# pinellolab/GRAFIMO

Hardware: AMD Instinct MI355X
Metric: scored haplotype k-mers/sec (higher is better)
Workload: dtype int32

## Files before the change

### grafimo_amd/_native.py

```python
import ctypes
import os

import numpy as np

_HERE = os.path.dirname(os.path.abspath(__file__))
LIB_PATH = os.environ.get("GRAFIMO_HIP_LIB") or os.path.join(_HERE, "csrc", "libgrafimo_hip.so")

GFM_OK = 0
GFM_ERR_INVALID = -1
GFM_ERR_ASSERT = -2
GFM_ERR_HIP = -3
GFM_ERR_NOMEM = -4
GFM_ERR_NODEVICE = -5
GFM_ERR_IO = -6
GFM_ERR_OVERFLOW = -7
GFM_NO_SELECT = 2**31 - 1
GFM_FLAG_RESET_HITS = 1
GFM_FLAG_CLEAR_HIST = 2
GFM_FLAG_CALLER_ORDERS_REUSE = 4
GFM_MAX_WIDTH = 64
GFM_BEST_ROW_BITS = 44
GFM_GRAPH_FORWARD_ONLY = 1
GFM_TSV_NO_NODEPATH = 1
GFM_WORKSPACE_RING = 4
GFM_HITS_DROP_ZERO_FREQ = 1
GFM_HITS_FIRST_PER_REGION = 2
GFM_VARIANT_ALL_SITES = 1
GFM_VARIANT_KEEP_ZERO_FREQ = 2
GFM_PAIRS_HAVE_OFFSETS = 1
GFM_LINKAGE_HAVE_OFFSETS = 1
GFM_SEQS_HAVE_LENGTHS = 1
ABI_VERSION = 12
RANGE = 1000

c_int = ctypes.c_int
c_i32 = ctypes.c_int32
c_i64 = ctypes.c_int64
c_u64 = ctypes.c_uint64
c_double = ctypes.c_double
c_void_p = ctypes.c_void_p
P = ctypes.POINTER

PROTOTYPES = {
    "gfm_abi_version": (c_int, []),
    "gfm_last_error": (ctypes.c_char_p, []),
    "gfm_device_count": (c_int, [P(c_int)]),
    "gfm_set_device": (c_int, [c_int]),
    "gfm_compute_log_odds": (c_int, [c_void_p, c_int, c_void_p, c_void_p]),
    "gfm_scale_pwm": (c_int, [c_void_p, c_int, c_void_p, P(c_int), P(c_int), P(c_int), P(c_double)]),
    "gfm_comp_pval_mat": (c_int, [c_void_p, c_int, c_void_p, c_void_p]),
    "gfm_comp_pval_mat_many": (c_int, [c_int, c_void_p, c_void_p, c_void_p, c_void_p]),
    "gfm_motif_create": (c_int, [c_void_p, c_int, c_void_p, c_int, c_int, c_double, c_void_p, P(c_void_p)]),
    "gfm_motif_create_many": (c_int, [c_int, c_void_p, c_void_p, c_void_p, c_void_p, c_void_p, c_void_p, c_void_p,
                                      c_void_p]),
    "gfm_motif_destroy": (None, [c_void_p]),
    "gfm_motif_width": (c_int, [c_void_p]),
    "gfm_motif_table_len": (c_int, [c_void_p]),
    "gfm_motif_score_range": (c_int, [c_void_p, P(c_i32), P(c_i32)]),
    "gfm_motif_tables": (c_int, [c_void_p, c_void_p, c_void_p]),
    "gfm_motif_pvalue_cutoff": (c_int, [c_void_p, c_double, P(c_i32)]),
    "gfm_motif_annotate": (c_int, [c_void_p, c_void_p, c_i64, c_void_p, c_void_p]),
    "gfm_score_kmers": (c_int, [c_void_p, c_void_p, c_i64, c_void_p, c_void_p, c_i32, c_i64,
                                c_void_p, c_i64, c_void_p, ctypes.c_uint32, c_void_p, c_void_p]),
    "gfm_score_kmers_multi": (c_int, [c_void_p, c_int, c_void_p, c_i64, c_void_p, c_void_p, c_void_p, c_i64,
                                      c_void_p, c_void_p, c_void_p, ctypes.c_uint32, c_void_p]),
    "gfm_score_kmers_multi_plan": (c_int, [c_void_p, c_int, c_void_p, c_void_p, c_void_p]),
    "gfm_profile_enable": (c_int, [c_void_p, c_int, c_int]),
    "gfm_profile_read": (c_int, [c_void_p, c_void_p, c_int, P(c_int)]),
    "gfm_profile_mark_tail": (c_int, [c_void_p, c_void_p]),
    "gfm_profile_read_tail": (c_int, [c_void_p, c_void_p, c_int, P(c_int)]),
    "gfm_calibrate_stream": (c_int, [c_int, c_i64, c_int, c_int, P(c_double), P(c_double)]),
    "gfm_qvalue_table": (c_int, [c_void_p, c_void_p, c_double, c_int, c_void_p, c_void_p, c_void_p,
                                 ctypes.c_uint32, c_void_p]),
    "gfm_qvalue_table_multi": (c_int, [c_void_p, c_int, c_void_p, c_double, c_int, c_void_p, c_void_p, c_void_p,
                                       ctypes.c_uint32, c_void_p]),
    "gfm_select_hits": (c_int, [c_void_p, c_void_p, c_i64, c_void_p, c_i64, c_void_p, c_i64, c_void_p,
                                ctypes.c_uint32, c_void_p]),
    "gfm_select_hits_from": (c_int, [c_void_p, c_void_p, c_i64, c_void_p, c_i64, c_void_p, c_i64, c_void_p,
                                     c_void_p, c_i64, c_void_p, c_void_p]),
    "gfm_region_ids": (c_int, [c_void_p, c_i32, c_i64, c_void_p, c_void_p]),
    "gfm_region_best": (c_int, [c_void_p, c_i64, c_void_p, c_i32, c_void_p, c_i32, c_void_p, c_i64, c_void_p, c_void_p]),
    "gfm_locus_max_workspace": (c_i64, [c_i64]),
    "gfm_locus_max": (c_int, [c_void_p, c_i64, c_void_p, c_i32, c_void_p, c_void_p, c_void_p, c_i32, c_void_p, c_void_p,
                              c_i64, c_void_p, c_void_p]),
    "gfm_scan_host": (c_int, [c_void_p, c_void_p, c_i64, c_double, c_int, c_int, c_i64, c_void_p,
                              c_void_p, c_void_p, c_void_p, c_void_p, P(c_i64)]),
    "gfm_tsv_open": (c_int, [P(ctypes.c_char_p), c_int, c_int, c_int, c_int, P(c_void_p), P(c_i64)]),
    "gfm_tsv_count_rows": (c_int, [ctypes.c_char_p, c_int, P(c_i64)]),
    "gfm_tsv_read": (c_int, [c_void_p] * 9),
    "gfm_tsv_name_count": (c_int, [c_void_p]),
    "gfm_tsv_names_bytes": (c_i64, [c_void_p]),
    "gfm_tsv_names": (c_int, [c_void_p, c_void_p, c_void_p]),
    "gfm_tsv_close": (None, [c_void_p]),
    "gfm_scan_tsv": (c_int, [c_void_p, P(ctypes.c_char_p), c_int, c_int, c_int, c_double, c_int, c_int, c_i64,
                             P(c_void_p), P(c_i64), P(c_i64)]),
    "gfm_scan_tsv_begin": (c_int, [c_void_p, c_int, P(ctypes.c_char_p), c_int, c_int, c_int, c_double, c_int, c_int,
                                   c_i64, c_void_p, P(c_void_p), P(c_i64)]),
    "gfm_scan_tsv_finish": (c_int, [c_void_p, c_void_p]),
# ... 174 lines not shown
```

### grafimo_amd/csrc/grafimo_hip.hip

```cpp

#include <hip/hip_runtime.h>

#include <algorithm>
#include <atomic>
#include <cmath>
#include <cstdarg>
#include <cstdint>
#include <cstdio>
#include <cstdlib>
#include <cstring>
#include <new>
#include <string>
#include <vector>

#include "grafimo_hip.h"

#define GFM_API extern "C" __attribute__((visibility("default")))

#include "gfm_hit_sort.hpp"
#include "gfm_common.hpp"
#include "gfm_score_kernels.hpp"
#include "gfm_quad_launch.hpp"
#include "gfm_stats_kernels.hpp"

// ... 7 lines not shown
    struct Window { int bins, lo; double mass; };
    std::vector<Window> windows;
    int device = 0;
    int n_cu = 256;
    int max_slabs = 0;
    int sel_slabs = 0;
    int reserve_cus = kReserveCUs;
    size_t lds_bytes = 0;
    std::vector<int64_t> sm;
    double bg[4] = {0, 0, 0, 0};
    std::vector<double> h_ptable;
    unsigned char *d_slab = nullptr;
    uint16_t *d_tab = nullptr;
    unsigned *d_ftab = nullptr;
    double *d_pmf = nullptr;
    double *d_ptable = nullptr;
    unsigned *d_partials[kWorkspaces] = {};
    unsigned *d_spill[kWorkspaces] = {};
    long long *d_resid[kWorkspaces] = {};
    int *d_resid_n[kWorkspaces] = {};
    QWork *d_qwork = nullptr;
    double *d_qscratch = nullptr;
    hipStream_t q_stream[kQStreams] = {};
    int q_streams_used = 0;
    unsigned long long q_last_use[kQStreams] = {}, q_calls = 0;
    hipEvent_t ev_selected = nullptr;
    hipStream_t sel_last_stream = nullptr;
    bool sel_valid = false;
    HitCtl *d_ctl = nullptr;
    unsigned call_no = 0;
    hipStream_t last_st = nullptr, last_tail = nullptr;
    unsigned same_pair_run = 0;
    hipEvent_t ev_scored[kWorkspaces] = {};
    hipEvent_t ev_posted[kWorkspaces] = {};
    bool posted_valid[kWorkspaces] = {};
    long long *d_sel_resid = nullptr;
    int *d_sel_resid_n = nullptr;
    HitCtl *d_sel_ctl = nullptr;
    unsigned sel_call_no = 0;
    std::vector<hipEvent_t> ev0, ev1;
    int ev_next = 0, ev_used = 0, ev_every = 1;
    unsigned ev_calls = 0;
    std::vector<hipEvent_t> tev0, tev1;
    int ev_last = -1;
    int tail_pending = -1;
    std::vector<int> tail_order;
};

namespace {

int ensure_device()
{
    int n = 0;
    hipError_t e = hipGetDeviceCount(&n);
    if (e != hipSuccess || n <= 0) {
        (void)hipGetLastError();
        return fail(GFM_ERR_NODEVICE, "no HIP device available (%s)",
                    e == hipSuccess ? "device count is 0" : hipGetErrorString(e));
    }
    return GFM_OK;
}

void cumulative_windows(const int64_t *sm, int W, std::vector<int> &lo, std::vector<int> &hi)
{
    lo.resize(W);
    hi.resize(W);
// ... 149 lines not shown
    q.hit_rows = d_hit_rows; q.hit_count = d_hit_count; q.hit_cap = cap;
    q.nslabs = hist_slabs; q.nb = win_nb; q.lo = win_lo; q.min_val = m->min_val;
    q.spill_lo = m->lo; q.spill_n = m->nb; q.hit_slabs = hit_slabs; q.par = ctl_slot;
    return q;
}

int launch_posts(const PostJob *jobs, int count, hipStream_t st)
{
    PostJobs all{};
    int live = 0, max_total = 0;
    for (int k = 0; k < count; ++k) {
        const PostJob &q = jobs[k];
        if (q.total == 0) {
            if (q.ctl)
                HIP_TRY(hipMemsetAsync(&q.ctl->mid[(q.par + kCtlAhead) % kCtlSlots], 0, sizeof(unsigned long long), st));
            continue;
        }
        all.j[live++] = q;
        max_total = std::max(max_total, q.total);
    }
    if (live == 0) return GFM_OK;
    hipLaunchKernelGGL(post_kernel, dim3((unsigned)max_total, (unsigned)live), dim3(256), 0, st, all);
    HIP_TRY(hipGetLastError());
    return GFM_OK;
}

int launch_post(gfm_motif *m, const unsigned *partials, int hist_slabs, unsigned long long *d_hist,
                int win_lo, int win_nb, unsigned *spill, const long long *resid, const int *resid_n, int hit_slabs, HitCtl *ctl, int ctl_slot,
                long long *d_hit_rows, long long cap, unsigned long long *d_hit_count, hipStream_t st)
{
    const PostJob q = post_job(m, partials, hist_slabs, d_hist, win_lo, win_nb, spill, resid, resid_n, hit_slabs, ctl,
                               ctl_slot, d_hit_rows, cap, d_hit_count);
    return launch_posts(&q, 1, st);
}

void fill_motif_args(MotifArgs &a, gfm_motif *m, int ws, int slot, int use_hist, int win_lo, int win_nb,
                     int cutoff,
                     int *d_scores, long long *d_hit_rows, long long cap,
                     const unsigned long long *d_hit_count_or_null)
{
    a.tab = m->d_tab;
    a.lo = win_lo;
    a.nb = win_nb;
    a.min_val = m->min_val;
    a.use_hist = use_hist;
    a.spill_lo = m->lo;
    a.spill_n = m->nb;
    a.spill = m->d_spill[ws];
    a.cutoff = cutoff;
    a.slot = slot;
    a.scores = d_scores;
    a.partials = m->d_partials[ws];
    a.hit_rows = d_hit_rows;
    a.hit_cap = cap;
    a.hit_count = d_hit_count_or_null;
    a.ctl = m->d_ctl;
    a.resid = m->d_resid[ws];
    a.resid_n = m->d_resid_n[ws];
}

bool plan_group(const gfm_motif_t *motifs, int n_left, const bool *with_hist, int *mm_out, int *waves_out,
                int *win_lo, int *win_nb)
{
    constexpr double kMinWindowMass = 0.999;
    const int W = motifs[0]->W;
    int mm = std::min(W <= kQuadMaxBatchWidth ? 3 : 1, n_left);
// ... 353 lines not shown
    double *rows = reinterpret_cast<double *>(d.p + rows_at), *pmfs = reinterpret_cast<double *>(d.p + pmf_at);
    size_t off = 0;
    for (DpJob &j : pk.jobs) {
        j.buf = rows + 2 * off;
        j.pmf = pmfs + off;
        off += (size_t)j.L;
    }
    img = pk.image();
    HIP_TRY(hipMemcpyAsync(d.p, img.data(), img.size(), hipMemcpyHostToDevice, nullptr));
    rc = pk.launch(d.p, n_motifs, false, nullptr);
    if (rc) return rc;
    HIP_TRY(hipMemcpy(h_pmf_out, pmfs, sizeof(double) * total_L, hipMemcpyDeviceToHost));
    return GFM_OK;
}

GFM_API int gfm_comp_pval_mat(const int64_t *sm, int W, const double *bg, double *h_pmf)
{
    return gfm_comp_pval_mat_many(1, sm, &W, bg, h_pmf);
}

GFM_API void gfm_motif_destroy(gfm_motif_t m)
{
    if (!m) return;
    if (m->d_slab) (void)hipFree(m->d_slab);
    for (int i = 0; i < kWorkspaces; ++i) {
        if (m->ev_scored[i]) (void)hipEventDestroy(m->ev_scored[i]);
        if (m->ev_posted[i]) (void)hipEventDestroy(m->ev_posted[i]);
    }
    for (auto e : m->ev0) (void)hipEventDestroy(e);
    for (auto e : m->ev1) (void)hipEventDestroy(e);
    for (auto e : m->tev0) (void)hipEventDestroy(e);
    for (auto e : m->tev1) (void)hipEventDestroy(e);
    if (m->ev_selected) (void)hipEventDestroy(m->ev_selected);
    delete m;
}

GFM_API int gfm_motif_create_many(int n_motifs, const int64_t *h_score_matrices, const int *widths, const double *h_bgs,
                                  const int *min_vals, const int *scales, const double *offsets,
                                  const double *const *h_pmfs, gfm_motif_t *out)
{
    if (n_motifs < 0) return fail(GFM_ERR_INVALID, "negative motif count %d", n_motifs);
    if (!out) return fail(GFM_ERR_INVALID, "NULL argument");
    for (int i = 0; i < n_motifs; ++i) out[i] = nullptr;
    if (n_motifs == 0) return GFM_OK;
    if (!h_score_matrices || !widths || !h_bgs || !min_vals || !scales || !offsets)
        return fail(GFM_ERR_INVALID, "NULL argument");
    std::vector<size_t> sm_at((size_t)n_motifs);
    size_t at = 0;
    for (int i = 0; i < n_motifs; ++i) {
        sm_at[(size_t)i] = at;
        const int rc = validate_motif(i, h_score_matrices + at, widths[i], h_bgs + 4 * (size_t)i, &min_vals[i], &scales[i]);
        if (rc) return rc;
        at += 4 * (size_t)widths[i];
    }
    int rc = ensure_device();
    if (rc) return rc;

    std::vector<std::vector<uint16_t>> tabs((size_t)n_motifs);
    std::vector<std::vector<unsigned>> ftabs((size_t)n_motifs);
    std::vector<unsigned char> img;
    DevBuf<unsigned char> d_pack;
    std::vector<gfm_motif *> ms((size_t)n_motifs, nullptr);
    auto bail = [&](int code) {
        (void)hipStreamSynchronize(nullptr);
        for (gfm_motif *m : ms) gfm_motif_destroy(m);
        return code;
// ... 82 lines not shown
        const int mid = (a + b) / 2;
        if (m->h_ptable[mid] < threshold) b = mid; else a = mid + 1;
    }
    *cutoff = a;
    return GFM_OK;
}

GFM_API int gfm_motif_annotate(gfm_motif_t m, const int32_t *scores, int64_t n, double *lo_out,
                               double *p_out)
{
    if (!m || (!scores && n)) return fail(GFM_ERR_INVALID, "NULL argument");
    for (int64_t i = 0; i < n; ++i) {
        const int s = scores[i];
        if (s < 0 || s >= m->L) return fail(GFM_ERR_INVALID, "score %d outside the table", s);
        if (lo_out) lo_out[i] = ((double)s / (double)m->scale) + ((double)m->W * m->offset);
        if (p_out) p_out[i] = m->h_ptable[s];
    }
    return GFM_OK;
}

GFM_API int gfm_score_kmers(gfm_motif_t m, const uint8_t *d_kmers, int64_t n, int32_t *d_scores,
                            uint64_t *d_hist, int32_t select_cutoff, int64_t row_base,
                            int64_t *d_hit_rows, int64_t hit_capacity, uint64_t *d_hit_count,
                            uint32_t flags, void *stream, void *tail_stream)
{
    if (!m) return fail(GFM_ERR_INVALID, "motif is NULL");
    if (n < 0) return fail(GFM_ERR_INVALID, "negative row count");
    hipStream_t st = static_cast<hipStream_t>(stream);
    hipStream_t tail = tail_stream ? static_cast<hipStream_t>(tail_stream) : st;
    const bool split = tail != st;
    if (n == 0) {
        if ((flags & GFM_FLAG_RESET_HITS) && d_hit_count) {
            if (split) {
                HIP_TRY(hipEventRecord(m->ev_scored[0], st));
                HIP_TRY(hipStreamWaitEvent(tail, m->ev_scored[0], 0));
            }
            HIP_TRY(hipMemsetAsync(d_hit_count, 0, sizeof(uint64_t), tail));
        }
        return GFM_OK;
    }
    if (!d_kmers) return fail(GFM_ERR_INVALID, "NULL device buffer");
    {
        int dev = -1;
        HIP_TRY(hipGetDevice(&dev));
        if (dev != m->device)
            return fail(GFM_ERR_INVALID, "the motif lives on device %d, the current device is %d", m->device, dev);
    }
    if ((reinterpret_cast<uintptr_t>(d_kmers) & 15u) != 0)
        return fail(GFM_ERR_INVALID, "d_kmers must be 16-byte aligned");
    if ((reinterpret_cast<uintptr_t>(d_scores) & 3u) != 0)
        return fail(GFM_ERR_INVALID, "d_scores must be 4-byte aligned");
    if (!d_scores && !d_hist && select_cutoff == GFM_NO_SELECT)
        return fail(GFM_ERR_INVALID, "nothing to do: no scores, no histogram, no selection");
    if (n > (int64_t)kQuadRows * 0x7fffff00ll)
        return fail(GFM_ERR_INVALID, "too many rows for one launch (split the batch)");
    const bool select = select_cutoff != GFM_NO_SELECT;
    if (select && (!d_hit_rows || !d_hit_count))
        return fail(GFM_ERR_INVALID, "selection requested without hit buffers");
    const int use_hist = d_hist ? 1 : 0;
    const long long nchunks = (n + kQuadRows - 1) / kQuadRows;
    const long long want = (nchunks + m->q_waves - 1) / m->q_waves;
    const int avail = split ? std::max(1, m->max_slabs - m->reserve_cus * (m->max_slabs / m->n_cu)) : m->max_slabs;
    int nslabs = (int)std::min<long long>(want, avail);
    if (want > avail) {
        long long best_cap = -1;
        for (int g = avail; g >= std::max(1, avail - avail / 8); --g) {
            const long long per_turn = (long long)g * m->q_waves;
            const long long cap = (nchunks + per_turn - 1) / per_turn * per_turn;
            if (best_cap < 0 || cap < best_cap) { best_cap = cap; nslabs = g; }
        }
#ifdef GFM_LAB
        if (const char *e = std::getenv("GRAFIMO_SCORE_GRID")) {
            const int g = atoi(e);
            if (g >= 1 && g <= m->max_slabs) nslabs = g;
        }
#endif
    }

    const unsigned k = m->call_no++;
    const int ws = (int)(k % (unsigned)kWorkspaces), slot = (int)(k % (unsigned)kCtlSlots);
    const int ws_prev = (int)((k + kWorkspaces - 1) % (unsigned)kWorkspaces);
    const bool reset = (flags & GFM_FLAG_RESET_HITS) != 0;
    const bool same_owner = st == m->last_st && tail == m->last_tail;
    const bool caller_orders = (flags & GFM_FLAG_CALLER_ORDERS_REUSE) && same_owner && m->same_pair_run >= (unsigned)kWorkspaces;
    m->same_pair_run = same_owner ? m->same_pair_run + 1 : 1;
    m->last_st = st;
    m->last_tail = tail;
    if (m->posted_valid[ws] && !caller_orders)
        HIP_TRY(hipStreamWaitEvent(st, m->ev_posted[ws], 0));
    if (split && select && !reset && m->posted_valid[ws_prev])
        HIP_TRY(hipStreamWaitEvent(st, m->ev_posted[ws_prev], 0));
    ScoreArgs<1> args{};
    args.store_through = d_scores ? score_store_through(n, 1) : 2;
    fill_motif_args(args.m[0], m, ws, slot, use_hist, m->hlo, m->hnb, select_cutoff, d_scores,
                    reinterpret_cast<long long *>(d_hit_rows), hit_capacity,
                    reset ? nullptr : reinterpret_cast<unsigned long long *>(d_hit_count));
    hipEvent_t scored = split ? m->ev_scored[ws] : nullptr;
    int rc = dispatch_quad(m->W, 1, m, d_kmers, n, row_base, &args, m->lds_bytes, nslabs, m->q_waves, st, false,
                           split ? &scored : nullptr);
    if (rc) return rc;
    if (split) HIP_TRY(hipStreamWaitEvent(tail, scored, 0));
    m->tail_pending = -1;
    if (split && m->ev_last >= 0 && !m->tev0.empty()) {
        HIP_TRY(hipEventRecord(m->tev0[m->ev_last], tail));
        m->tail_pending = m->ev_last;
    }
    rc = launch_post(m, m->d_partials[ws], nslabs, reinterpret_cast<unsigned long long *>(d_hist),
                     m->hlo, m->hnb, m->d_spill[ws], m->d_resid[ws], m->d_resid_n[ws], select ? nslabs : 0, m->d_ctl, slot,
                     reinterpret_cast<long long *>(d_hit_rows), hit_capacity,
                     reinterpret_cast<unsigned long long *>(d_hit_count), tail);
    if (rc) return rc;
    if (split) {
        HIP_TRY(hipEventRecord(m->ev_posted[ws], tail));
        m->posted_valid[ws] = true;
    } else {
        m->posted_valid[ws] = false;
    }
    return GFM_OK;
}

GFM_API int gfm_score_kmers_multi(const gfm_motif_t *motifs, int n_motifs, const uint8_t *d_kmers,
                                  int64_t n, int32_t *const *d_scores, uint64_t *const *d_hist,
                                  const int32_t *select_cutoffs, int64_t row_base,
                                  int64_t *const *d_hit_rows, const int64_t *hit_capacity,
                                  uint64_t *const *d_hit_count, uint32_t flags, void *stream)
{
    if (!motifs || n_motifs < 1) return fail(GFM_ERR_INVALID, "NULL argument");
    if (n < 0) return fail(GFM_ERR_INVALID, "negative row count");
    hipStream_t st = static_cast<hipStream_t>(stream);
    const bool reset = (flags & GFM_FLAG_RESET_HITS) != 0;
    bool no_scores = d_scores == nullptr;
    if (d_scores) {
        int n_null = 0;
// ... 27 lines not shown
        if ((reinterpret_cast<uintptr_t>(d_scores[i]) & 3u) != 0)
            return fail(GFM_ERR_INVALID, "d_scores[%d] must be 4-byte aligned", i);
    const int W = motifs[0]->W;
    const long long nchunks = (n + kQuadRows - 1) / kQuadRows;

    int i = 0;
    while (i < n_motifs) {
        int mm = 0, waves = kWavesPerWG, nb_lds[3] = {0, 0, 0};
        int win_lo[3] = {0, 0, 0}, win_nb[3] = {0, 0, 0};
        bool with_hist[3];
        for (int k = 0; k < 3; ++k) with_hist[k] = i + k < n_motifs && d_hist && d_hist[i + k];
        if (!plan_group(motifs + i, n_motifs - i, with_hist, &mm, &waves, win_lo, win_nb))
            return fail(GFM_ERR_INVALID, "no LDS left for a histogram window at width %d", W);
        for (int k = 0; k < mm; ++k) {
            if (win_nb[k] > motifs[i + k]->part_nb)
                return fail(GFM_ERR_INVALID, "internal error: histogram window larger than the workspace");
            nb_lds[k] = (d_hist && d_hist[i + k]) ? win_nb[k] + 1 : 0;
        }
        size_t lds = quad_fixed_lds(W, waves, mm);
        for (int k = 0; k < mm; ++k) lds += sizeof(unsigned) * (size_t)nb_lds[k];
        const long long want = (nchunks + waves - 1) / waves;
        int nslabs = (int)std::min<long long>(want, motifs[i]->max_slabs);
        for (int k = 1; k < mm; ++k) nslabs = std::min(nslabs, motifs[i + k]->max_slabs);
        int ws[3], slot[3], uh[3];
        ScoreArgs<1> a1{};
        ScoreArgs<2> a2{};
        ScoreArgs<3> a3{};
        a1.store_through = a2.store_through = a3.store_through = no_scores ? 2 : score_store_through(n, mm);
        for (int k = 0; k < mm; ++k) {
            gfm_motif *mo = motifs[i + k];
            const unsigned c = mo->call_no++;
            mo->same_pair_run = 0;
            mo->last_st = mo->last_tail = nullptr;
            ws[k] = (int)(c % (unsigned)kWorkspaces);
            slot[k] = (int)(c % (unsigned)kCtlSlots);
            mo->posted_valid[ws[k]] = false;
            uh[k] = (d_hist && d_hist[i + k]) ? 1 : 0;
            const int cut = select_cutoffs ? select_cutoffs[i + k] : GFM_NO_SELECT;
            const bool sel = cut != GFM_NO_SELECT;
            MotifArgs &dst = mm == 1 ? a1.m[k] : (mm == 2 ? a2.m[k] : a3.m[k]);
            fill_motif_args(dst, mo, ws[k], slot[k], uh[k], win_lo[k], win_nb[k], cut, no_scores ? nullptr : d_scores[i + k],
                            sel ? reinterpret_cast<long long *>(d_hit_rows[i + k]) : nullptr,
                            sel ? hit_capacity[i + k] : 0,
                            (sel && !reset) ? reinterpret_cast<const unsigned long long *>(d_hit_count[i + k])
                                            : nullptr);
        }
        const void *args = mm == 1 ? static_cast<const void *>(&a1) : (mm == 2 ? static_cast<const void *>(&a2) : &a3);
        int rc = dispatch_quad(W, mm, motifs[i], d_kmers, n, row_base, args, lds, nslabs, waves, st, false);
        if (rc) return rc;
        PostJob posts[kPostJobs];
        for (int k = 0; k < mm; ++k) {
            gfm_motif *mo = motifs[i + k];
            const int cut = select_cutoffs ? select_cutoffs[i + k] : GFM_NO_SELECT;
            const bool sel = cut != GFM_NO_SELECT;
            posts[k] = post_job(mo, mo->d_partials[ws[k]], nslabs,
                                uh[k] ? reinterpret_cast<unsigned long long *>(d_hist[i + k]) : nullptr,
                                win_lo[k], win_nb[k], mo->d_spill[ws[k]], mo->d_resid[ws[k]], mo->d_resid_n[ws[k]],
                                sel ? nslabs : 0, mo->d_ctl, slot[k],
                                sel ? reinterpret_cast<long long *>(d_hit_rows[i + k]) : nullptr,
                                sel ? hit_capacity[i + k] : 0,
                                sel ? reinterpret_cast<unsigned long long *>(d_hit_count[i + k]) : nullptr);
        }
        rc = launch_posts(posts, mm, st);
        if (rc) return rc;
        i += mm;
    }
    return GFM_OK;
}

GFM_API int gfm_score_kmers_multi_plan(const gfm_motif_t *motifs, int n_motifs, const int32_t *with_hist,
                                       int32_t *group_size_out, int32_t *waves_out)
{
    if (!motifs || n_motifs < 1) return fail(GFM_ERR_INVALID, "NULL argument");
    for (int i = 0; i < n_motifs; ++i) {
        if (!motifs[i]) return fail(GFM_ERR_INVALID, "motif %d is NULL", i);
        if (motifs[i]->W != motifs[0]->W)
            return fail(GFM_ERR_INVALID, "motifs of one batched launch must share their width (%d vs %d)",
                        motifs[i]->W, motifs[0]->W);
    }
    int i = 0;
    while (i < n_motifs) {
        int mm = 0, waves = 0, win_lo[3], win_nb[3];
        bool wh[3];
        for (int k = 0; k < 3; ++k) wh[k] = i + k < n_motifs && (!with_hist || with_hist[i + k]);
        if (!plan_group(motifs + i, n_motifs - i, wh, &mm, &waves, win_lo, win_nb))
            return fail(GFM_ERR_INVALID, "no LDS left for a histogram window at width %d", motifs[0]->W);
        for (int k = 0; k < mm; ++k) {
            if (group_size_out) group_size_out[i + k] = mm;
            if (waves_out) waves_out[i + k] = waves;
        }
        i += mm;
    }
    return GFM_OK;
}

GFM_API int gfm_profile_enable(gfm_motif_t m, int slots, int every)
{
    if (!m || slots < 0 || every < 1) return fail(GFM_ERR_INVALID, "bad argument");
    m->ev_every = every;
    m->ev_calls = 0;
    for (auto e : m->ev0) (void)hipEventDestroy(e);
    for (auto e : m->ev1) (void)hipEventDestroy(e);
    for (auto e : m->tev0) (void)hipEventDestroy(e);
    for (auto e : m->tev1) (void)hipEventDestroy(e);
    m->ev0.clear();
    m->ev1.clear();
    m->tev0.clear();
    m->tev1.clear();
    m->tail_order.clear();
    m->ev_next = m->ev_used = 0;
    m->ev_last = m->tail_pending = -1;
    for (int i = 0; i < slots; ++i) {
        hipEvent_t a, b, c, d;
        HIP_TRY(hipEventCreate(&a));
        HIP_TRY(hipEventCreate(&b));
        HIP_TRY(hipEventCreate(&c));
        HIP_TRY(hipEventCreate(&d));
        m->ev0.push_back(a);
        m->ev1.push_back(b);
        m->tev0.push_back(c);
        m->tev1.push_back(d);
    }
    return GFM_OK;
}

GFM_API int gfm_profile_mark_tail(gfm_motif_t m, void *stream)
{
    if (!m) return fail(GFM_ERR_INVALID, "motif is NULL");
    if (m->tail_pending < 0) return GFM_OK;
    HIP_TRY(hipEventRecord(m->tev1[m->tail_pending], static_cast<hipStream_t>(stream)));
    if ((int)m->tail_order.size() < (int)m->tev0.size()) m->tail_order.push_back(m->tail_pending);
    m->tail_pending = -1;
    return GFM_OK;
// ... 324 lines not shown
```

### grafimo_amd/device.py

```python
import ctypes
from collections import OrderedDict
from typing import List, Optional

import numpy as np

from . import _native as nv

RANGE = nv.RANGE


def _torch():
    import torch
    return torch


_FP_WEIGHTS = {}


def _fingerprint(pmf) -> tuple:
    words = np.ascontiguousarray(pmf, dtype=np.float64).view(np.uint64)
    n = len(words)
    if not n:
        return (0, 0, 0)
    w = _FP_WEIGHTS.get(n)
    if w is None:
        if len(_FP_WEIGHTS) > 64:
            _FP_WEIGHTS.clear()
        w = _FP_WEIGHTS[n] = np.arange(n, dtype=np.uint64) * np.uint64(0x9E3779B97F4A7C15) + np.uint64(1) | np.uint64(1)
    return (n, int(np.bitwise_xor.reduce(words)), int((words * w).sum(dtype=np.uint64)))


class DeviceMotif:

    def __init__(self, score_matrix, bg, min_val, scale, offset, pmf: Optional[np.ndarray] = None):
        sm, bg, pmf = self._set_numbers(score_matrix, bg, min_val, scale, offset, pmf)
        h = ctypes.c_void_p()
        nv.check(nv.lib().gfm_motif_create(nv.ptr(sm), self.width, nv.ptr(bg), self.min_val,
                                           self.scale, self.offset, nv.ptr(pmf), ctypes.byref(h)))
        self._adopt(h)

    def _set_numbers(self, score_matrix, bg, min_val, scale, offset, pmf):
        sm = np.ascontiguousarray(score_matrix, dtype=np.int64)
        if sm.ndim != 2 or sm.shape[0] != 4:
            raise ValueError("score_matrix must be [4, W]")
        bg = np.ascontiguousarray(bg, dtype=np.float64)
        self.score_matrix = sm
        self.width = int(sm.shape[1])
        self.L = RANGE * self.width + 1
        self.min_val = int(min_val)
        self.scale = int(scale)
        self.offset = float(offset)
        if pmf is not None:
            pmf = np.ascontiguousarray(pmf, dtype=np.float64)
            if pmf.shape != (self.L,):
                raise ValueError(f"pval_matrix must have {self.L} entries")
        return sm, bg, pmf

    def _adopt(self, h):
        self._h = h
        lo, hi = ctypes.c_int32(), ctypes.c_int32()
        nv.check(nv.lib().gfm_motif_score_range(self._h, ctypes.byref(lo), ctypes.byref(hi)))
        self.score_lo, self.score_hi = lo.value, hi.value

    @staticmethod
    def _numbers_of(motif, use_motif_pmf=True):
        from .motif import dense_bg, dense_score_matrix
        pmf = getattr(motif, "pval_matrix", None) if use_motif_pmf else None
        return (dense_score_matrix(motif), dense_bg(motif), int(motif.min_val), int(motif.scale), float(motif.offset), pmf)

    @classmethod
    def from_motif(cls, motif, use_motif_pmf=True):
        return cls(*cls._numbers_of(motif, use_motif_pmf))

    @classmethod
    def create_many(cls, motifs, use_motif_pmf=True) -> List["DeviceMotif"]:
        return cls._create_many([cls._numbers_of(m, use_motif_pmf) for m in motifs])

    @classmethod
    def _create_many(cls, specs) -> List["DeviceMotif"]:
        M = len(specs)
        if M == 0:
            return []
        dms = [cls.__new__(cls) for _ in range(M)]
        arrays = [dm._set_numbers(*spec) for dm, spec in zip(dms, specs)]
        if any(bg.shape != (4,) for _, bg, _ in arrays):
            raise ValueError("bg must hold 4 probabilities")
        sm_all = np.concatenate([sm.ravel() for sm, _, _ in arrays])
        widths = np.array([dm.width for dm in dms], dtype=np.int32)
        bgs = np.ascontiguousarray(np.stack([bg for _, bg, _ in arrays]))
        min_vals = np.array([dm.min_val for dm in dms], dtype=np.int32)
        scales = np.array([dm.scale for dm in dms], dtype=np.int32)
        offsets = np.array([dm.offset for dm in dms], dtype=np.float64)
        pmfs = (ctypes.c_void_p * M)(*[nv.ptr(pmf) for _, _, pmf in arrays])
        hs = (ctypes.c_void_p * M)()
        nv.check(nv.lib().gfm_motif_create_many(M, nv.ptr(sm_all), nv.ptr(widths), nv.ptr(bgs), nv.ptr(min_vals),
# ... 154 lines not shown
                     stream=None, clear_hist=False):
        nv.check(nv.lib().gfm_qvalue_table(
            self._h, hist.data_ptr(), float(threshold), int(bool(on_qvalue)),
            qtable.data_ptr() if qtable is not None else None,
            cutoff.data_ptr() if cutoff is not None else None,
            nrows.data_ptr() if nrows is not None else None,
            nv.GFM_FLAG_CLEAR_HIST if clear_hist else 0, _stream_ptr(stream)))

    def select_hits(self, scores, cutoff, hit_rows, hit_count, row_base=0, stream=None,
                    reset_hits=False):
        n = int(scores.numel())
        nv.check(nv.lib().gfm_select_hits(self._h, scores.data_ptr() if n else None, n, cutoff.data_ptr(),
                                          int(row_base), hit_rows.data_ptr(), int(hit_rows.numel()),
                                          hit_count.data_ptr(),
                                          nv.GFM_FLAG_RESET_HITS if reset_hits else 0,
                                          _stream_ptr(stream)))

    def select_hits_from(self, scores, cutoff, cand_rows, cand_count, hit_rows, hit_count, row_base=0, stream=None):
        n = int(scores.numel())
        nv.check(nv.lib().gfm_select_hits_from(self._h, scores.data_ptr() if n else None, n, cutoff.data_ptr(),
                                               int(row_base), cand_rows.data_ptr(), int(cand_rows.numel()),
                                               cand_count.data_ptr(), hit_rows.data_ptr(), int(hit_rows.numel()),
                                               hit_count.data_ptr(), _stream_ptr(stream)))

    def profile_enable(self, slots: int, every: int = 1):
        nv.check(nv.lib().gfm_profile_enable(self._h, int(slots), int(every)))

    def profile_read(self, capacity: int = 4096):
        ms = np.empty(capacity, dtype=np.float32)
        n = ctypes.c_int(0)
        nv.check(nv.lib().gfm_profile_read(self._h, nv.ptr(ms), capacity, ctypes.byref(n)))
        return ms[: n.value].copy()

    def profile_mark_tail(self, stream=None):
        nv.check(nv.lib().gfm_profile_mark_tail(self._h, _stream_ptr(stream)))

    def profile_read_tail(self, capacity: int = 4096):
        ms = np.empty(capacity, dtype=np.float32)
        n = ctypes.c_int(0)
        nv.check(nv.lib().gfm_profile_read_tail(self._h, nv.ptr(ms), capacity, ctypes.byref(n)))
        return ms[: n.value].copy()

    def scan_host(self, kmers: np.ndarray, threshold: float, on_qvalue=False, want_qvalues=True,
                  capacity: Optional[int] = None):
        kmers = np.ascontiguousarray(kmers, dtype=np.uint8)
        n = int(kmers.shape[0])
        if n and kmers.shape[1] != self.width:
            raise ValueError("k-mer width differs from the motif width")
        cap = n if capacity is None else int(capacity)
        while True:
            rows = np.empty(cap, dtype=np.int64)
            sc = np.empty(cap, dtype=np.int32)
            lo = np.empty(cap, dtype=np.float64)
            pv = np.empty(cap, dtype=np.float64)
            qv = np.empty(cap, dtype=np.float64) if want_qvalues else None
            nh = ctypes.c_int64(0)
            rc = nv.lib().gfm_scan_host(self._h, nv.ptr(kmers) if n else None, n, float(threshold),
                                        int(bool(on_qvalue)), int(bool(want_qvalues)), cap,
                                        nv.ptr(rows), nv.ptr(sc), nv.ptr(lo), nv.ptr(pv),
                                        nv.ptr(qv), ctypes.byref(nh))
            if rc == nv.GFM_ERR_OVERFLOW and nh.value > cap:
                cap = int(nh.value)
                continue
            nv.check(rc)
            break
        k = nh.value
# ... 101 lines not shown
```

### grafimo_amd/scan.py

```python
from typing import Optional

import numpy as np

from . import _native as _nv
from .device import DeviceMotif, _torch

HIT_SCORE_BITS = 20


def score_ring_step(turn: int, n_slots: int, n_arrays: int, tail_reads):
    array = turn % n_arrays
    oldest = max(0, turn - n_slots + 1)
    w = turn - n_arrays
    while w >= oldest:
        if tail_reads(w):
            return array, w
        w -= n_arrays
    return array, None


class ScanSlot:

    def __init__(self, dm: DeviceMotif, n_rows: int, hit_capacity: int, device, scores=None):
        torch = _torch()
        self.n_rows = int(n_rows)
        self.hit_capacity = int(hit_capacity)
        self.scores = scores if scores is not None else torch.empty(self.n_rows, dtype=torch.int32, device=device)
        self.hist = torch.zeros(dm.L, dtype=torch.int64, device=device)
        self.qtable = torch.empty(dm.L, dtype=torch.float64, device=device)
        self.cutoff = torch.zeros(1, dtype=torch.int32, device=device)
        self.nrows = torch.zeros(1, dtype=torch.int64, device=device)
        self.hits = torch.zeros(self.hit_capacity + 1, dtype=torch.int64, device=device)
        self.best = None
        self.cand = None
        self.p_cand_count = self.p_cand_rows = None
        self.done = torch.cuda.Event()
        self.tail_done = torch.cuda.Event()
        self.used = False
        self.reads_scores = False
        self.gathered = None
        self.p_scores = self.scores.data_ptr()
        self.p_hist = self.hist.data_ptr()
        self.p_qtable = self.qtable.data_ptr()
        self.p_cutoff = self.cutoff.data_ptr()
        self.p_nrows = self.nrows.data_ptr()
        self.p_hit_count = self.hits.data_ptr()
        self.p_hit_rows = self.hits.data_ptr() + 8

    def candidates(self):
        if self.cand is None:
            self.cand = _torch().zeros_like(self.hits)
            self.p_cand_count = self.cand.data_ptr()
            self.p_cand_rows = self.cand.data_ptr() + 8
        return self.cand

    @property
    def hit_count(self):
        return self.hits[:1]

    @property
    def hit_rows(self):
        return self.hits[1:]


class KmerScanner:
    def __init__(self, dm: DeviceMotif, n_rows: int, hit_capacity: Optional[int] = None,
                 device=None, group=None, n_slots: int = 3, side_stream: bool = True,
                 always_collective: bool = False, gather_group=None, host_paced: Optional[bool] = None,
                 candidates: bool = True, score_buffers: Optional[int] = None):
        torch = _torch()
        self.dm = dm
        self.device = device if device is not None else torch.device("cuda", torch.cuda.current_device())
        self.group = group
        self.world = 1
        self.rank = 0
        if group is not None or (torch.distributed.is_available() and torch.distributed.is_initialized()):
            self.world = torch.distributed.get_world_size(group)
            self.rank = torch.distributed.get_rank(group)
        self.collective = self.world > 1 or (always_collective and torch.distributed.is_initialized())
        self._gather_ok = True
        self.gather_group = gather_group if gather_group is not None else group
        self._gather_stream = None
        self.tail_done = None
        if self.collective and side_stream:
            self._gather_stream = torch.cuda.Stream(device=self.device, priority=-1)
        cap = int(hit_capacity) if hit_capacity is not None else int(n_rows)
        nb = n_slots if score_buffers is None else max(1, min(int(score_buffers), n_slots))
        ring = [torch.empty(int(n_rows), dtype=torch.int32, device=self.device) for _ in range(nb)]
        self.slots = [ScanSlot(dm, n_rows, cap, self.device, scores=ring[k % nb]) for k in range(n_slots)]
        self._ring = ring
        self._ring_p = [a.data_ptr() for a in ring]
        self._score_ring = nb
        self.side = torch.cuda.Stream(device=self.device, priority=-1) if side_stream else None
        self._side_p = self.side.cuda_stream if self.side is not None else None
        self._lib = _nv.lib()
        self._cutoffs = {}
        self.host_paced = (n_slots >= 3) if host_paced is None else bool(host_paced)
        if self.host_paced and n_slots < 2:
            raise ValueError("host-paced slot reuse needs at least two slots")
        self._reuse_flag = _nv.GFM_FLAG_CALLER_ORDERS_REUSE if n_slots <= _nv.GFM_WORKSPACE_RING else 0
        self.candidates = bool(candidates)
        self.profile_tail = False
        self._turn = 0
        self.gather_len = cap + 1
        self._regions = None
        self.top_only = False

    def set_regions(self, region, n_regions: int, freq=None, top_only: bool = False):
        torch = _torch()
        assert region.dtype == torch.int32 and region.is_cuda
        self._regions = (region, int(n_regions), freq)
        self.top_only = bool(top_only)
        for s in self.slots:
            s.best = torch.zeros(int(n_regions), dtype=torch.int64, device=self.device)
            s.gathered = None

    def size_gather(self, margin: float = 1.25, granule: int = 512) -> int:
        torch = _torch()
        self.finish()
        torch.cuda.synchronize(self.device)
        m = torch.stack([s.hits[0] for s in self.slots]).max().reshape(1)
        if self.collective:
            torch.distributed.all_reduce(m, op=torch.distributed.ReduceOp.MAX, group=self.group)
        want = int(int(m.item()) * margin) + 1
        want = -(-want // granule) * granule
        self.gather_len = min(self.slots[0].hit_capacity, want) + 1
        for s in self.slots:
            s.gathered = None
        return self.gather_len

    def enqueue(self, d_kmers, threshold: float, on_qvalue: bool = False, want_qvalues: bool = True,
                row_base: int = 0, gather_hits: bool = False) -> ScanSlot:
        if on_qvalue and not want_qvalues:
            raise ValueError("q-value threshold without q-values")
        torch = _torch()
        lib = self._lib
        dm = self.dm
        turn, n_slots = self._turn, len(self.slots)
        slot = self.slots[turn % n_slots]
        self._turn += 1
        main = torch.cuda.current_stream(self.device)
        main_p = main.cuda_stream
        tail = self.side if self.side is not None else main
        tail_p = self._side_p if self.side is not None else main_p
        if slot.used:
            if self.host_paced:
                slot.done.synchronize()
            else:
                main.wait_event(slot.done)
        slot.used = True
        if self._score_ring < n_slots:
            a, wait = score_ring_step(turn, n_slots, self._score_ring, self._turn_reads_scores)
            if wait is not None:
                if self.host_paced:
                    self.slots[wait % n_slots].done.synchronize()
                else:
                    main.wait_event(self.slots[wait % n_slots].done)
            slot.scores, slot.p_scores = self._ring[a], self._ring_p[a]
            slot.reads_scores = on_qvalue or self._regions is not None
        n = int(d_kmers.shape[0])
        kp = d_kmers.data_ptr() if n else None
        h = dm.handle
        use_cand = on_qvalue and self.candidates
        if not on_qvalue:
            key = float(threshold)
            cut = self._cutoffs.get(key)
            if cut is None:
                cut = self._cutoffs[key] = dm.pvalue_cutoff(key)
            _nv.check(lib.gfm_score_kmers(h, kp, n, slot.p_scores, slot.p_hist if want_qvalues else None,
                                          cut, int(row_base), slot.p_hit_rows, slot.hit_capacity,
                                          slot.p_hit_count, _nv.GFM_FLAG_RESET_HITS | self._reuse_flag, main_p, tail_p))
        elif not use_cand:
            _nv.check(lib.gfm_score_kmers(h, kp, n, slot.p_scores, slot.p_hist, _nv.GFM_NO_SELECT, 0,
                                          None, 0, None, self._reuse_flag, main_p, tail_p))
        else:
            key = float(threshold)
            cut = self._cutoffs.get(key)
            if cut is None:
                cut = self._cutoffs[key] = dm.pvalue_cutoff(key)
            slot.candidates()
            _nv.check(lib.gfm_score_kmers(h, kp, n, slot.p_scores, slot.p_hist, cut, int(row_base),
                                          slot.p_cand_rows, slot.hit_capacity, slot.p_cand_count,
                                          _nv.GFM_FLAG_RESET_HITS | self._reuse_flag, main_p, tail_p))
        if want_qvalues:
            if self.collective:
                with torch.cuda.stream(tail):
                    torch.distributed.all_reduce(slot.hist, group=self.group)
            _nv.check(lib.gfm_qvalue_table(h, slot.p_hist, float(threshold), int(bool(on_qvalue)),
                                           slot.p_qtable, slot.p_cutoff, slot.p_nrows,
                                           _nv.GFM_FLAG_CLEAR_HIST, tail_p))
        if on_qvalue and not use_cand:
            _nv.check(lib.gfm_select_hits(h, slot.p_scores, n, slot.p_cutoff, int(row_base),
                                          slot.p_hit_rows, slot.hit_capacity, slot.p_hit_count,
                                          _nv.GFM_FLAG_RESET_HITS, tail_p))
        elif on_qvalue:
            _nv.check(lib.gfm_select_hits_from(h, slot.p_scores, n, slot.p_cutoff, int(row_base),
                                               slot.p_cand_rows, slot.hit_capacity, slot.p_cand_count,
                                               slot.p_hit_rows, slot.hit_capacity, slot.p_hit_count, tail_p))
        if self._regions is not None:
            region, n_regions, freq = self._regions
            with torch.cuda.stream(tail):
                slot.best.zero_()
            _nv.check(lib.gfm_region_best(slot.p_scores, n, region.data_ptr(), n_regions,
                                          freq.data_ptr() if freq is not None else None,
                                          0 if on_qvalue else self._cutoffs[float(threshold)],
                                          slot.p_cutoff if on_qvalue else None, int(row_base), slot.best.data_ptr(), tail_p))
        if gather_hits and self.collective:
            gs = self._gather_stream
            if gs is not None:
                slot.tail_done.record(tail)
                gs.wait_event(slot.tail_done)
                with torch.cuda.stream(gs):
                    self._gather(slot)
                if self.profile_tail:
                    lib.gfm_profile_mark_tail(h, gs.cuda_stream)
                slot.done.record(gs)
# ... 190 lines not shown
```

### include/grafimo_hip.h

```cpp
#ifndef GRAFIMO_HIP_H
#define GRAFIMO_HIP_H

#include <stdint.h>

#ifdef __cplusplus
extern "C" {
#endif

#define GFM_ABI_VERSION 12

#define GFM_OK 0
#define GFM_ERR_INVALID (-1)
#define GFM_ERR_ASSERT (-2)
#define GFM_ERR_HIP (-3)
#define GFM_ERR_NOMEM (-4)
#define GFM_ERR_NODEVICE (-5)
#define GFM_ERR_IO (-6)
#define GFM_ERR_OVERFLOW (-7)

#define GFM_MAX_WIDTH 64
#define GFM_NO_SELECT INT32_MAX
#define GFM_FLAG_RESET_HITS 1u
#define GFM_FLAG_CLEAR_HIST 2u
#define GFM_FLAG_CALLER_ORDERS_REUSE 4u
#define GFM_WORKSPACE_RING 4
#define GFM_HIT_SCORE_BITS 20

int gfm_abi_version(void);
const char *gfm_last_error(void);
int gfm_device_count(int *count);
int gfm_set_device(int ordinal);

int gfm_compute_log_odds(const double *h_probs, int width, const double *h_bg,
                         double *h_logodds_out);

int gfm_scale_pwm(const double *h_logodds, int width, int64_t *h_score_matrix_out,
                  int *min_val, int *max_val, int *scale, double *offset);

int gfm_comp_pval_mat(const int64_t *h_score_matrix, int width, const double *h_bg,
                      double *h_pmf_out);
int gfm_comp_pval_mat_many(int n_motifs, const int64_t *h_score_matrices, const int *widths,
                           const double *h_bgs, double *h_pmf_out);

typedef struct gfm_motif *gfm_motif_t;

int gfm_motif_create(const int64_t *h_score_matrix, int width, const double *h_bg,
                     int min_val, int scale, double offset, const double *h_pmf,
                     gfm_motif_t *out);
int gfm_motif_create_many(int n_motifs, const int64_t *h_score_matrices, const int *widths,
                          const double *h_bgs, const int *min_vals, const int *scales,
                          const double *offsets, const double *const *h_pmfs, gfm_motif_t *out);
void gfm_motif_destroy(gfm_motif_t m);
int gfm_motif_width(gfm_motif_t m);
int gfm_motif_table_len(gfm_motif_t m);
int gfm_motif_score_range(gfm_motif_t m, int32_t *lo, int32_t *hi);
int gfm_motif_tables(gfm_motif_t m, double *h_pmf_out, double *h_ptable_out);
int gfm_motif_pvalue_cutoff(gfm_motif_t m, double threshold, int32_t *cutoff);
int gfm_motif_annotate(gfm_motif_t m, const int32_t *h_scores, int64_t n,
                       double *h_logodds_out, double *h_pvalue_out);

int gfm_score_kmers(gfm_motif_t m, const uint8_t *d_kmers, int64_t n, int32_t *d_scores,
                    uint64_t *d_hist, int32_t select_cutoff, int64_t row_base,
                    int64_t *d_hit_rows, int64_t hit_capacity, uint64_t *d_hit_count,
                    uint32_t flags, void *stream, void *tail_stream);

int gfm_score_kmers_multi(const gfm_motif_t *motifs, int n_motifs, const uint8_t *d_kmers,
                          int64_t n, int32_t *const *d_scores, uint64_t *const *d_hist,
                          const int32_t *select_cutoffs, int64_t row_base,
                          int64_t *const *d_hit_rows, const int64_t *hit_capacity,
                          uint64_t *const *d_hit_count, uint32_t flags, void *stream);

int gfm_score_kmers_multi_plan(const gfm_motif_t *motifs, int n_motifs, const int32_t *with_hist,
                               int32_t *group_size_out, int32_t *waves_out);

int gfm_profile_enable(gfm_motif_t m, int slots, int every);
int gfm_profile_read(gfm_motif_t m, float *h_ms_out, int capacity, int *n_out);
int gfm_profile_mark_tail(gfm_motif_t m, void *stream);
int gfm_profile_read_tail(gfm_motif_t m, float *h_ms_out, int capacity, int *n_out);

int gfm_calibrate_stream(int loads_per_store, int64_t in_bytes, int store_policy, int launches,
                         double *us_per_launch, double *bytes_per_launch);

int gfm_qvalue_table(gfm_motif_t m, uint64_t *d_hist, double threshold, int on_qvalue,
                     double *d_qtable_out, int32_t *d_cutoff_out, uint64_t *d_nrows_out,
                     uint32_t flags, void *stream);
int gfm_qvalue_table_multi(const gfm_motif_t *motifs, int n_motifs, uint64_t *const *d_hist,
                           double threshold, int on_qvalue, double *const *d_qtable_out,
                           int32_t *const *d_cutoff_out, uint64_t *const *d_nrows_out, uint32_t flags,
                           void *stream);

int gfm_select_hits(gfm_motif_t m, const int32_t *d_scores, int64_t n, const int32_t *d_cutoff,
                    int64_t row_base, int64_t *d_hit_rows, int64_t hit_capacity,
                    uint64_t *d_hit_count, uint32_t flags, void *stream);
int gfm_select_hits_from(gfm_motif_t m, const int32_t *d_scores, int64_t n, const int32_t *d_cutoff,
                         int64_t row_base, const int64_t *d_cand_rows, int64_t cand_capacity,
                         const uint64_t *d_cand_count, int64_t *d_hit_rows, int64_t hit_capacity,
                         uint64_t *d_hit_count, void *stream);

#define GFM_BEST_ROW_BITS 44
int gfm_region_ids(const int64_t *d_region_off, int32_t n_regions, int64_t n, int32_t *d_region_out, void *stream);
int gfm_region_best(const int32_t *d_scores, int64_t n, const int32_t *d_region, int32_t n_regions,
                    const int64_t *d_freq, int32_t min_score, const int32_t *d_cutoff, int64_t row_base,
                    uint64_t *d_best, void *stream);
// ... 220 lines not shown
```

Baseline: 228.4 billion.

## Overlap consecutive score launches on alternating side streams

Adds an overlap mode where host-paced scoring calls in caller-ordered reuse mode launch the scoring kernel on one of two private non-blocking streams, alternating per call, instead of the caller's stream. This lets back-to-back batches run concurrently rather than serialising on the main stream. Joins back to the caller stream are inserted when overlap is off or on reset/multi paths. When overlapping, the grid is capped to the available slabs. It adds stream/event bookkeeping and a hipStreamQuery idle check per call, and risks ordering bugs if the join events are missed.

```diff
diff --git a/grafimo_amd/_native.py b/grafimo_amd/_native.py
--- a/grafimo_amd/_native.py
+++ b/grafimo_amd/_native.py
@@ -18,6 +18,7 @@
 GFM_FLAG_RESET_HITS = 1
 GFM_FLAG_CLEAR_HIST = 2
 GFM_FLAG_CALLER_ORDERS_REUSE = 4
+GFM_FLAG_OVERLAP_LAUNCHES = 8
 GFM_MAX_WIDTH = 64
 GFM_BEST_ROW_BITS = 44
 GFM_GRAPH_FORWARD_ONLY = 1
@@ -64,6 +65,8 @@
                                 c_void_p, c_i64, c_void_p, ctypes.c_uint32, c_void_p, c_void_p]),
     "gfm_score_kmers_multi": (c_int, [c_void_p, c_int, c_void_p, c_i64, c_void_p, c_void_p, c_void_p, c_i64,
                                       c_void_p, c_void_p, c_void_p, ctypes.c_uint32, c_void_p]),
+    "gfm_overlapped_launches": (c_int, [c_void_p, P(c_u64)]),
+    "gfm_motif_set_overlap": (c_int, [c_void_p, c_int]),
     "gfm_score_kmers_multi_plan": (c_int, [c_void_p, c_int, c_void_p, c_void_p, c_void_p]),
     "gfm_profile_enable": (c_int, [c_void_p, c_int, c_int]),
     "gfm_profile_read": (c_int, [c_void_p, c_void_p, c_int, P(c_int)]),
diff --git a/grafimo_amd/csrc/grafimo_hip.hip b/grafimo_amd/csrc/grafimo_hip.hip
--- a/grafimo_amd/csrc/grafimo_hip.hip
+++ b/grafimo_amd/csrc/grafimo_hip.hip
@@ -63,6 +63,12 @@
     hipStream_t last_st = nullptr, last_tail = nullptr;
     unsigned same_pair_run = 0;
     hipEvent_t ev_scored[kWorkspaces] = {};
+    hipStream_t launch_st[2] = {};
+    hipEvent_t launch_last[2] = {};
+    hipEvent_t ev_join[kWorkspaces] = {};
+    unsigned quiet = 0;
+    bool overlap_on = true;
+    unsigned long long overlapped = 0;
     hipEvent_t ev_posted[kWorkspaces] = {};
     bool posted_valid[kWorkspaces] = {};
     long long *d_sel_resid = nullptr;
@@ -278,6 +284,49 @@
     const PostJob q = post_job(m, partials, hist_slabs, d_hist, win_lo, win_nb, spill, resid, resid_n, hit_slabs, ctl,
                                ctl_slot, d_hit_rows, cap, d_hit_count);
     return launch_posts(&q, 1, st);
+}
+
+int join_launch_streams(gfm_motif *m, hipStream_t st)
+{
+    for (int i = 0; i < 2; ++i) {
+        if (!m->launch_last[i]) continue;
+        HIP_TRY(hipStreamWaitEvent(st, m->launch_last[i], 0));
+        m->launch_last[i] = nullptr;
+    }
+    return GFM_OK;
+}
+
+__global__ void launch_stream_warm_kernel() {}
+
+int ensure_launch_streams(gfm_motif *m)
+{
+    for (int i = 0; i < 2; ++i) {
+        if (m->launch_st[i]) continue;
+        HIP_TRY(hipStreamCreateWithFlags(&m->launch_st[i], hipStreamNonBlocking));
+        hipLaunchKernelGGL(launch_stream_warm_kernel, dim3(1), dim3(kWave), 0, m->launch_st[i]);
+        HIP_TRY(hipGetLastError());
+    }
+    for (int i = 0; i < kWorkspaces; ++i)
+        if (!m->ev_join[i]) HIP_TRY(hipEventCreateWithFlags(&m->ev_join[i], hipEventDisableTiming));
+    return GFM_OK;
+}
+
+int caller_stream_idle(gfm_motif *m, hipStream_t st, bool *idle)
+{
+    *idle = false;
+    if (m->quiet) {
+        --m->quiet;
+        return GFM_OK;
+    }
+    const hipError_t q = hipStreamQuery(st);
+    if (q != hipSuccess) {
+        (void)hipGetLastError();
+        if (q != hipErrorNotReady) HIP_TRY(q);
+        m->quiet = 3;
+        return GFM_OK;
+    }
+    *idle = true;
+    return GFM_OK;
 }
 
 void fill_motif_args(MotifArgs &a, gfm_motif *m, int ws, int slot, int use_hist, int win_lo, int win_nb,
@@ -697,6 +746,10 @@
     for (auto e : m->tev0) (void)hipEventDestroy(e);
     for (auto e : m->tev1) (void)hipEventDestroy(e);
     if (m->ev_selected) (void)hipEventDestroy(m->ev_selected);
+    for (int i = 0; i < 2; ++i)
+        if (m->launch_st[i]) (void)hipStreamDestroy(m->launch_st[i]);
+    for (int i = 0; i < kWorkspaces; ++i)
+        if (m->ev_join[i]) (void)hipEventDestroy(m->ev_join[i]);
     delete m;
 }
 
@@ -845,6 +898,8 @@
     if (n == 0) {
         if ((flags & GFM_FLAG_RESET_HITS) && d_hit_count) {
             if (split) {
+                const int rcj = join_launch_streams(m, st);
+                if (rcj) return rcj;
                 HIP_TRY(hipEventRecord(m->ev_scored[0], st));
                 HIP_TRY(hipStreamWaitEvent(tail, m->ev_scored[0], 0));
             }
@@ -882,12 +937,6 @@
             const long long cap = (nchunks + per_turn - 1) / per_turn * per_turn;
             if (best_cap < 0 || cap < best_cap) { best_cap = cap; nslabs = g; }
         }
-#ifdef GFM_LAB
-        if (const char *e = std::getenv("GRAFIMO_SCORE_GRID")) {
-            const int g = atoi(e);
-            if (g >= 1 && g <= m->max_slabs) nslabs = g;
-        }
-#endif
     }
 
     const unsigned k = m->call_no++;
@@ -896,9 +945,36 @@
     const bool reset = (flags & GFM_FLAG_RESET_HITS) != 0;
     const bool same_owner = st == m->last_st && tail == m->last_tail;
     const bool caller_orders = (flags & GFM_FLAG_CALLER_ORDERS_REUSE) && same_owner && m->same_pair_run >= (unsigned)kWorkspaces;
+    const bool orders_next = (flags & GFM_FLAG_CALLER_ORDERS_REUSE) && same_owner && m->same_pair_run + 1 == (unsigned)kWorkspaces;
     m->same_pair_run = same_owner ? m->same_pair_run + 1 : 1;
     m->last_st = st;
     m->last_tail = tail;
+    bool overlap = false, idle = false;
+    if ((flags & GFM_FLAG_OVERLAP_LAUNCHES) && split && m->overlap_on && !(select && !reset) &&
+        (caller_orders || orders_next)) {
+        int rco = ensure_launch_streams(m);
+        if (!rco && caller_orders) {
+            overlap = true;
+            rco = caller_stream_idle(m, st, &idle);
+        }
+        if (rco) return rco;
+    }
+    hipStream_t kst = overlap ? m->launch_st[k & 1u] : st;
+    if (overlap && !idle) {
+        HIP_TRY(hipEventRecord(m->ev_join[ws], st));
+        HIP_TRY(hipStreamWaitEvent(kst, m->ev_join[ws], 0));
+    }
+    if (overlap && want > avail) nslabs = avail;
+#ifdef GFM_LAB
+    if (const char *e = std::getenv("GRAFIMO_SCORE_GRID")) {
+        const int g = atoi(e);
+        if (want > avail && g >= 1 && g <= m->max_slabs) nslabs = g;
+    }
+#endif
+    if (!overlap) {
+        const int rcj = join_launch_streams(m, st);
+        if (rcj) return rcj;
+    }
     if (m->posted_valid[ws] && !caller_orders)
         HIP_TRY(hipStreamWaitEvent(st, m->ev_posted[ws], 0));
     if (split && select && !reset && m->posted_valid[ws_prev])
@@ -909,9 +985,13 @@
                     reinterpret_cast<long long *>(d_hit_rows), hit_capacity,
                     reset ? nullptr : reinterpret_cast<unsigned long long *>(d_hit_count));
     hipEvent_t scored = split ? m->ev_scored[ws] : nullptr;
-    int rc = dispatch_quad(m->W, 1, m, d_kmers, n, row_base, &args, m->lds_bytes, nslabs, m->q_waves, st, false,
+    int rc = dispatch_quad(m->W, 1, m, d_kmers, n, row_base, &args, m->lds_bytes, nslabs, m->q_waves, kst, false,
                            split ? &scored : nullptr);
     if (rc) return rc;
+    if (overlap) {
+        m->launch_last[k & 1u] = scored;
+        if (idle) ++m->overlapped;
+    }
     if (split) HIP_TRY(hipStreamWaitEvent(tail, scored, 0));
     m->tail_pending = -1;
     if (split && m->ev_last >= 0 && !m->tev0.empty()) {
@@ -1005,6 +1085,7 @@
             const unsigned c = mo->call_no++;
             mo->same_pair_run = 0;
             mo->last_st = mo->last_tail = nullptr;
+            if (const int rcj = join_launch_streams(mo, st)) return rcj;
             ws[k] = (int)(c % (unsigned)kWorkspaces);
             slot[k] = (int)(c % (unsigned)kCtlSlots);
             mo->posted_valid[ws[k]] = false;
@@ -1067,11 +1148,30 @@
     return GFM_OK;
 }
 
+GFM_API int gfm_motif_set_overlap(gfm_motif_t m, int enabled)
+{
+    if (!m) return fail(GFM_ERR_INVALID, "motif is NULL");
+    m->overlap_on = enabled != 0;
+    return GFM_OK;
+}
+
+GFM_API int gfm_overlapped_launches(gfm_motif_t m, uint64_t *count)
+{
+    if (!m || !count) return fail(GFM_ERR_INVALID, "NULL argument");
+    *count = m->overlapped;
+    return GFM_OK;
+}
+
 GFM_API int gfm_profile_enable(gfm_motif_t m, int slots, int every)
 {
     if (!m || slots < 0 || every < 1) return fail(GFM_ERR_INVALID, "bad argument");
     m->ev_every = every;
     m->ev_calls = 0;
+    for (int i = 0; i < 2; ++i) {
+        if (!m->launch_last[i]) continue;
+        HIP_TRY(hipEventSynchronize(m->launch_last[i]));
+        m->launch_last[i] = nullptr;
+    }
     for (auto e : m->ev0) (void)hipEventDestroy(e);
     for (auto e : m->ev1) (void)hipEventDestroy(e);
     for (auto e : m->tev0) (void)hipEventDestroy(e);
diff --git a/grafimo_amd/device.py b/grafimo_amd/device.py
--- a/grafimo_amd/device.py
+++ b/grafimo_amd/device.py
@@ -1,4 +1,5 @@
 import ctypes
+import os
 from collections import OrderedDict
 from typing import List, Optional
 
@@ -61,6 +62,8 @@
         lo, hi = ctypes.c_int32(), ctypes.c_int32()
         nv.check(nv.lib().gfm_motif_score_range(self._h, ctypes.byref(lo), ctypes.byref(hi)))
         self.score_lo, self.score_hi = lo.value, hi.value
+        if os.environ.get("GRAFIMO_SCORE_OVERLAP", "").strip() == "0":
+            self.set_overlap(False)
 
     @staticmethod
     def _numbers_of(motif, use_motif_pmf=True):
@@ -281,6 +284,14 @@
         nv.check(nv.lib().gfm_profile_read(self._h, nv.ptr(ms), capacity, ctypes.byref(n)))
         return ms[: n.value].copy()
 
+    def set_overlap(self, enabled: bool):
+        nv.check(nv.lib().gfm_motif_set_overlap(self._h, int(bool(enabled))))
+
+    def overlapped_launches(self) -> int:
+        n = ctypes.c_uint64(0)
+        nv.check(nv.lib().gfm_overlapped_launches(self._h, ctypes.byref(n)))
+        return int(n.value)
+
     def profile_mark_tail(self, stream=None):
         nv.check(nv.lib().gfm_profile_mark_tail(self._h, _stream_ptr(stream)))
 
diff --git a/grafimo_amd/scan.py b/grafimo_amd/scan.py
--- a/grafimo_amd/scan.py
+++ b/grafimo_amd/scan.py
@@ -1,3 +1,4 @@
+import os
 from typing import Optional
 
 import numpy as np
@@ -17,6 +18,17 @@
             return array, w
         w -= n_arrays
     return array, None
+
+
+OVERLAP_LAUNCHES_DEFAULT = True
+
+
+def overlap_launches(host_paced: bool, side_stream: bool, collective: bool, n_slots: int, env: Optional[str] = None) -> bool:
+    if not (host_paced and side_stream) or collective or n_slots > _nv.GFM_WORKSPACE_RING:
+        return False
+    if env is not None and env.strip() in ("0", "1"):
+        return env.strip() == "1"
+    return OVERLAP_LAUNCHES_DEFAULT
 
 
 class ScanSlot:
@@ -39,6 +51,7 @@
         self.used = False
         self.reads_scores = False
         self.gathered = None
+        self.kmers = None
         self.p_scores = self.scores.data_ptr()
         self.p_hist = self.hist.data_ptr()
         self.p_qtable = self.qtable.data_ptr()
@@ -99,8 +112,13 @@
         if self.host_paced and n_slots < 2:
             raise ValueError("host-paced slot reuse needs at least two slots")
         self._reuse_flag = _nv.GFM_FLAG_CALLER_ORDERS_REUSE if n_slots <= _nv.GFM_WORKSPACE_RING else 0
+        self.overlap = overlap_launches(self.host_paced, side_stream, self.collective, n_slots,
+                                        os.environ.get("GRAFIMO_SCORE_OVERLAP"))
+        if self.overlap:
+            self._reuse_flag |= _nv.GFM_FLAG_OVERLAP_LAUNCHES
         self.candidates = bool(candidates)
         self.profile_tail = False
+        self.overlap_qvalue_batches = False
         self._turn = 0
         self.gather_len = cap + 1
         self._regions = None
@@ -149,6 +167,8 @@
             else:
                 main.wait_event(slot.done)
         slot.used = True
+        if self.overlap:
+            slot.kmers = d_kmers
         if self._score_ring < n_slots:
             a, wait = score_ring_step(turn, n_slots, self._score_ring, self._turn_reads_scores)
             if wait is not None:
@@ -162,6 +182,9 @@
         kp = d_kmers.data_ptr() if n else None
         h = dm.handle
         use_cand = on_qvalue and self.candidates
+        reuse_flag = self._reuse_flag
+        if on_qvalue and not self.overlap_qvalue_batches:
+            reuse_flag &= ~_nv.GFM_FLAG_OVERLAP_LAUNCHES
         if not on_qvalue:
             key = float(threshold)
             cut = self._cutoffs.get(key)
@@ -169,10 +192,10 @@
                 cut = self._cutoffs[key] = dm.pvalue_cutoff(key)
             _nv.check(lib.gfm_score_kmers(h, kp, n, slot.p_scores, slot.p_hist if want_qvalues else None,
                                           cut, int(row_base), slot.p_hit_rows, slot.hit_capacity,
-                                          slot.p_hit_count, _nv.GFM_FLAG_RESET_HITS | self._reuse_flag, main_p, tail_p))
+                                          slot.p_hit_count, _nv.GFM_FLAG_RESET_HITS | reuse_flag, main_p, tail_p))
         elif not use_cand:
             _nv.check(lib.gfm_score_kmers(h, kp, n, slot.p_scores, slot.p_hist, _nv.GFM_NO_SELECT, 0,
-                                          None, 0, None, self._reuse_flag, main_p, tail_p))
+                                          None, 0, None, reuse_flag, main_p, tail_p))
         else:
             key = float(threshold)
             cut = self._cutoffs.get(key)
@@ -181,7 +204,7 @@
             slot.candidates()
             _nv.check(lib.gfm_score_kmers(h, kp, n, slot.p_scores, slot.p_hist, cut, int(row_base),
                                           slot.p_cand_rows, slot.hit_capacity, slot.p_cand_count,
-                                          _nv.GFM_FLAG_RESET_HITS | self._reuse_flag, main_p, tail_p))
+                                          _nv.GFM_FLAG_RESET_HITS | reuse_flag, main_p, tail_p))
         if want_qvalues:
             if self.collective:
                 with torch.cuda.stream(tail):
diff --git a/include/grafimo_hip.h b/include/grafimo_hip.h
--- a/include/grafimo_hip.h
+++ b/include/grafimo_hip.h
@@ -24,6 +24,7 @@
 #define GFM_FLAG_CLEAR_HIST 2u
 #define GFM_FLAG_CALLER_ORDERS_REUSE 4u
 #define GFM_WORKSPACE_RING 4
+#define GFM_FLAG_OVERLAP_LAUNCHES 8u
 #define GFM_HIT_SCORE_BITS 20
 
 int gfm_abi_version(void);
@@ -69,6 +70,9 @@
                           const int32_t *select_cutoffs, int64_t row_base,
                           int64_t *const *d_hit_rows, const int64_t *hit_capacity,
                           uint64_t *const *d_hit_count, uint32_t flags, void *stream);
+
+int gfm_overlapped_launches(gfm_motif_t m, uint64_t *count);
+int gfm_motif_set_overlap(gfm_motif_t m, int enabled);
 
 int gfm_score_kmers_multi_plan(const gfm_motif_t *motifs, int n_motifs, const int32_t *with_hist,
                                int32_t *group_size_out, int32_t *waves_out);
```

New measurement: 240.7 billion, median of 6. 1.05x the previous value.
